# viiika/Diffusion-Conductor

Hardware: AMD Instinct MI355X
Metric: motion frames/sec (DDIM-50, 60s clip, bs=32 per GPU) (higher is better)
Workload: dtype f16; 1 GPU; configs[1]: DDIM-50 sampling loop, bs=32 clips/GPU x 1800 frames (60 s), linear attention, precision=fp16, conditioning + x_T resident in HBM (loop-only); clips_per_gpu=32, frames_per_clip=1800, ddim_steps=50, parallelism=clip-dp1, precise_tail_steps=1

## Files before the change

### diffusion-conductor_amd/csrc/dc_api.hip

```cpp
#include <hip/hip_runtime.h>

#include <algorithm>
#include <cmath>
#include <cstdarg>
#include <cstdio>
#include <cstdlib>
#include <cstring>
#include <map>
#include <string>
#include <tuple>
#include <vector>

#include "../../include/dc_ddim.h"
#include "dc_common.h"
#include "dc_form.h"
#include "dc_launch.h"
#include "dc_music.h"
#include "dc_pack.h"

namespace {

thread_local std::string g_err;

int fail(int code, const char* fmt, ...) {
// ... 639 lines not shown
int enqueue_step(dc_sampler* s, hipStream_t st, const Step& c, const Switches& w, StepDone* done = nullptr) {
    static const bool want_stamps = getenv("DC_STAMPS") != nullptr;
    const int B = s->B, T = s->T, M = s->M, G = s->G, Tx = s->Tx;
    const StepForm f = step_form(Geometry{B, T, Tx, G, s->num_cu, s->cap_rec_floats}, settings_of(s), w, c, want_stamps);
    const bool folded = f.folded;
    const int fs = f.fs, ff = f.ff, graph_step = c.graph_step;
    const bool ss = f.ss, sf = s->split_film;
    const unsigned l16_tag = folded ? 16u * (unsigned)graph_step : (0x40000000u | (16u * (s->l16_seq++ & 0x3ffffffu)));
    if (!f.error.empty()) return fail(DC_ERR_INVALID, "%s", f.error.c_str());
    if (done) done->embedded_next = f.embed_next, done->folded = folded;
    const DcModel* dmod = (c.split && !s->split_small) ? s->d_model_split : s->d_model;
    const int* iter_base = folded ? s->d_iter : nullptr;
    const int* t_src = folded ? s->d_t_of_iter + graph_step : s->d_t_clip;
    const float* coef_src = folded ? s->d_coef_of_iter + DC_COEF * (size_t)graph_step : s->d_coef_cur;
    const int* snap_src = folded ? s->d_snap_of_iter + graph_step : s->d_snap_cur;
    if (c.loop_mode && !folded)
        LAUNCH(K_BEGIN, dc_launch_begin_step(st, s->d_iter, s->d_t_of_iter, s->d_coef_of_t, s->d_snap_of_iter,
                                             s->d_t_clip, s->d_coef_cur, s->d_snap_cur, B));
    if (c.loop_mode && (s->upd_flags & DC_UPD_ZSTEP))
        LAUNCH(K_NOISE, dc_launch_step_noise(st, s->d_zstep, (size_t)B * Tx * s->cfg.input_feats, 0, reinterpret_cast<const unsigned long long*>(s->d_zslot) + 1,
                                             iter_base, folded ? graph_step : 0,
                                             folded ? nullptr : s->d_snap_cur, 0));
    if (!f.fuse_silu)
        LAUNCH(K_SILU, dc_launch_silu_emb(st, ff, sf, s->d_pp, s->h_model.temb, s->d_t_clip, s->d_s_hi, s->d_s_lo, G, T, B));
    DcEmbedArgs ea{};
    if (f.fuse_embed) ea = DcEmbedArgs{dmod, c.x_src, s->d_h, s->d_recs, s->d_length, M, Tx, f.nwg, f.upc, ss ? 1 : 0, 0};
    if (f.fuse_extra) ea = DcEmbedArgs{s->d_model, c.x_src, s->d_h, s->d_recs, s->d_length, M, Tx, f.nwg, f.upc, 0, 1};
    DcFilmArgs fa = film_args(s, f.fuse_silu ? s->d_pp : nullptr, t_src);
    if (f.g1_tiles) fa.bias_ft = s->h_model.film_b_g1, fa.bias16 = s->h_model.film_b16_g1;
    if (f.film_tail) fa.W16 = s->h_model.film_w16_tail;
    fa.clk = want_stamps ? s->d_stamps + 252 : nullptr;
    if (f.adapt) fa.rate_in = s->d_film_rate + 1024 * s->film_rate_parity, fa.rate_out = s->d_film_rate + 1024 * (s->film_rate_parity ^ 1);
    fa.iter_base = iter_base;
    fa.embed = (f.fuse_embed || f.fuse_extra) ? &ea : nullptr;
    const bool diag_skip_film = getenv("DC_DIAG_SKIP_FILM") && !f.fuse_embed && !f.fuse_extra && s->diag_film_done;
    s->diag_film_done = true;
    if (!diag_skip_film) LAUNCH(K_FILM, dc_launch_film_gemm(st, ff, sf, fa));
    s->film_rate_parity ^= 1;
    const int nl_run = f.nl_run;
    DcLayerArgs la{};
    la.dm = dmod, la.hbuf = s->d_h, la.E = s->d_E, la.NT = s->NT, la.recs = s->d_recs, la.length = s->d_length, la.xin = c.x_src, la.xout = c.x_dst;
    la.out_mode = c.loop_mode ? 1 : 0, la.coef_cur = coef_src, la.snap_cur = snap_src, la.snaps = s->d_snaps, la.iter_base = iter_base;
    la.M = M, la.T = T, la.G = G, la.B = B, la.Tx = Tx;
    la.upd = DcUpdate{s->d_zslot, s->d_status, (c.loop_mode ? s->upd_flags : 0) | f.upd_flags, folded ? graph_step : -1, nullptr};
    DcLayerArgs la_stamps = la;
    la_stamps.upd.stamps = s->d_stamps;
    if (s->cfg.no_eff) {
        LAUNCH(K_EMBED, dc_launch_embed_front_full(st, fs, ss, dmod, c.x_src, s->d_h, s->d_kv_sa[0], M, T, B, s->KT));
        for (int l = 0; l < nl_run; ++l)
            LAUNCH(K_LAYER, dc_launch_layer_full(st, fs, ss, (want_stamps && l == 3) ? la_stamps : la, l, s->d_kv_sa[l & 1], s->d_kv_sa[(l + 1) & 1],
                                                 s->d_kv_ca, s->KT, (l == nl_run - 1) ? f.stop_stage : 0));
        return DC_OK;
    }
    const DcLayerForm lf{fs, ss, f.wgr, f.narrow, f.g1_tiles, f.upc, f.rec_stride};
    if (f.fuse_embed || f.fuse_extra || c.embedded) {
    } else if (c.dbg.first >= 0)
        LAUNCH(K_EMBED, dc_launch_front_from_h(st, fs, ss, dmod, s->d_h, s->d_recs, s->d_length, M, T, G, B, c.dbg.first));
    else
        LAUNCH(K_EMBED, dc_launch_embed_front(st, lf, dmod, c.x_src, s->d_h, s->d_recs, s->d_length, M, T, G, B,
                                              want_stamps ? s->d_stamps + 256 : nullptr, Tx));
    for (int l = c.dbg.first >= 0 ? c.dbg.first : 0; l < nl_run; ++l) {
        if (f.layer16) {
            static const bool stamps16 = getenv("DC_L16_STAMPS") != nullptr;
            LAUNCH(K_LAYER, dc_launch_layer16(st, fs, (stamps16 && l == 3) ? la_stamps : la, l, s->d_a_ca16, f.upc16, f.rec_stride,
                                              l == 0 ? f.upc_narrow : f.upc16, l == 0 ? (size_t)2 * DC_REC_FLOATS : (size_t)DC_REC_FLOATS,
                                              f.l16_shared ? s->d_gran : nullptr, l16_tag, f.g1_tiles));
// ... 758 lines not shown
```

### diffusion-conductor_amd/csrc/dc_form.h

```cpp
#pragma once
#include <algorithm>
#include <cstdio>
#include <cstdlib>
#include <optional>
#include <string>

#include "dc_common.h"

constexpr int DCF_BF16 = 0, DCF_MIXED = 1, DCF_BF16X3 = 2, DCF_FP16 = 3;

struct Formats {
    int small_fmt = 0, film_fmt = 0;
    bool split_small = false, split_film = false;
    void set_precision(int precision) {
        split_small = precision == DCF_MIXED || precision == DCF_BF16X3;
        split_film = precision == DCF_BF16X3;
        small_fmt = precision == DCF_FP16 ? 1 : 0;
        film_fmt = (precision == DCF_FP16 || precision == DCF_MIXED) ? 1 : 0;
    }
};

#define DC_FORM_SWITCHES(X)                                                                                                            \
    X(no_wgrec, "DC_NO_WGREC") X(no_narrow, "DC_NO_NARROW") X(no_align, "DC_NO_ALIGN") X(align, "DC_ALIGN")                          \
    X(no_fuse_embed, "DC_NO_FUSE_EMBED") X(film_static, "DC_FILM_STATIC") X(begin_step, "DC_BEGIN_STEP") X(no_pad, "DC_NO_PAD")      \
    X(no_layer16, "DC_NO_LAYER16") X(l16_own_combine, "DC_L16_OWN_COMBINE") X(l16_test_drop_slice, "DC_L16_TEST_DROP_SLICE")         \
    X(tail_film_bf16, "DC_TAIL_FILM_BF16") X(flat_units, "DC_FLAT_UNITS") X(no_embed_next, "DC_NO_EMBED_NEXT")
struct Switches {
#define X(field, name) bool field = false;
    DC_FORM_SWITCHES(X)
#undef X
    static Switches read() {
        Switches w;
#define X(field, name) w.field = getenv(name) != nullptr;
        DC_FORM_SWITCHES(X)
#undef X
        return w;
    }
    unsigned long long bits() const {
        unsigned long long k = 0;
        int i = 0;
#define X(field, name) k |= (field ? 1ull : 0ull) << i++;
        DC_FORM_SWITCHES(X)
#undef X
        return k;
    }
};

inline size_t rec_capacity(size_t g) { return std::max(g * 2, 4 * ((g + 3) / 4) + 8) * DC_REC_FLOATS; }

struct Geometry {
    int B = 0, T = 0, Tx = 0, G = 0;
    int num_cu = 0;
    size_t cap_rec_floats = 0;
};

struct Settings {
    int precision = DCF_FP16;
    Formats fmt;
    bool no_eff = false;
    int clip_aligned = -1;
    bool l16_own = false;
    int num_layers = 0;
    bool split_model = false;
    bool film_w16 = false, film_w16_tail = false;
    int l16_max_units = 0;
};

struct Hooks {
    int layers = -1, stage = 0;
    int first = -1;
    bool production() const { return layers < 0 && stage == 0 && first < 0; }
};

struct StepOpts {
    bool loop_mode = false;
    int graph_step = -1;
    bool split = false;
    bool g1_loop = false;
    bool next_plain = false;
    bool embedded = false;
    bool profile = false;
    Hooks dbg;
};

struct StepForm {
    std::string error;
    bool ss = false;
    bool film_tail = false;
    int fs = 0, ff = 0;
    bool fuse_silu = false;
    bool folded = false;
    bool adapt = false;
    bool wgr = false, narrow = false, aligned = false, layer16 = false, l16_shared = false;
    int upc = 0, upc16 = 0, upc_narrow = 0, nwg = 0;
    size_t rec_stride = 0;
    bool mixed_form = false, embed_next = false, fuse_embed = false, fuse_extra = false, g1_tiles = false;
    int upd_flags = 0;
    int nl_run = 0, stop_stage = 0;
};

inline bool can_split_steps(const Settings& s, const Hooks& dbg) {
    return (s.precision == DCF_FP16 || s.precision == DCF_BF16) && dbg.production() && s.split_model;
}

inline StepForm step_form(const Geometry& g, const Settings& s, const Switches& w, const StepOpts& o, bool stamps) {
    StepForm f;
    const int B = g.B, T = g.T, G = g.G;
    const Hooks& dbg = o.dbg;
    const bool quiet = dbg.production() && !stamps;
    const bool ss = f.ss = s.fmt.split_small || o.split, sf = s.fmt.split_film;
    f.film_tail = o.split && !s.fmt.split_small && s.film_w16_tail && !w.tail_film_bf16;
    const int fs = f.fs = s.fmt.small_fmt, ff = f.ff = f.film_tail ? 1 : s.fmt.film_fmt;
    const bool fuse_silu = f.fuse_silu = !sf && dbg.layers < 0;
    f.folded = o.loop_mode && o.graph_step >= 0 && fuse_silu && !s.no_eff && !w.begin_step && dbg.stage == 0;
    f.adapt = !w.film_static && g.num_cu <= 1024;
    f.nl_run = (dbg.layers >= 0 && dbg.layers < s.num_layers) ? dbg.layers : s.num_layers;
    f.stop_stage = s.no_eff ? (dbg.stage ? dbg.stage : (f.nl_run < s.num_layers ? 3 : 0)) : dbg.stage;
    const bool wgr = f.wgr = T >= 256 && !w.no_wgrec && dbg.first < 0 && !s.no_eff && (!ss || (T % 32 == 0 && dbg.production() && !w.no_align));
    const bool can_align = wgr && T % 32 == 0 && !w.no_align;
    const int upc_wide = (T + 255) / 256, upc_narrow = f.upc_narrow = (T + 127) / 128;
    const bool aligned_env = can_align && w.align;
    const int nwg_narrow = can_align ? B * upc_narrow : (G + 3) / 4;
    const bool narrow = f.narrow = wgr && !ss && nwg_narrow <= g.num_cu && T <= 3840 && quiet && !w.no_narrow;
    const int nwg_flat = (G + 7) / 8, ncu = g.num_cu > 0 ? g.num_cu : 256;
    const bool same_rounds = ((long long)B * upc_wide + ncu - 1) / ncu == ((long long)nwg_flat + ncu - 1) / ncu;
    const bool aligned_wide = s.clip_aligned > 0 || aligned_env || (s.clip_aligned < 0 && same_rounds && !w.flat_units);
    const bool aligned = f.aligned = can_align && (narrow || ss || aligned_wide);
    const int upc16 = f.upc16 = (T + 63) / 64;
    const bool layer16 = f.layer16 = narrow && aligned && (long long)B * upc16 <= g.num_cu && upc16 <= s.l16_max_units && dbg.first < 0 && !w.no_layer16;
    const int upc = f.upc = aligned ? (narrow ? upc_narrow : upc_wide) : 0;
    const int nwg = f.nwg = aligned ? B * upc : (narrow ? (G + 3) / 4 : (G + 7) / 8);
    f.l16_shared = layer16 && !s.l16_own && !w.l16_own_combine;
    f.rec_stride = wgr ? (size_t)nwg * 2 * DC_REC_FLOATS : 0;
    const size_t rec_floats = wgr ? 2 * f.rec_stride : (size_t)G * 2 * DC_REC_FLOATS;
    if (rec_floats > g.cap_rec_floats) {
        char buf[160];
        snprintf(buf, sizeof buf, "unit records of this launch form (%zu floats) exceed the workspace (%zu)", rec_floats, g.cap_rec_floats);
        f.error = buf;
        return f;
    }
    const bool mixed_form = f.mixed_form = ss && !sf && ff == 1 && fs == 0;
    const bool wide_plain = wgr && !narrow && !ss && fuse_silu && ff == fs && quiet && !s.no_eff;
    f.embed_next = !w.no_embed_next && o.loop_mode && o.next_plain && wide_plain;
    if (o.embedded && !(o.loop_mode && wide_plain)) {
        f.error = "internal: a step whose front work was done by its predecessor changed its launch form";
        return f;
    }
    f.fuse_embed = !o.embedded && wgr && !narrow && (ss ? (aligned && mixed_form) : ff == fs) && fuse_silu && quiet && nwg <= g.num_cu &&
// ... 50 lines not shown
```

### diffusion-conductor_amd/csrc/dc_kernels.hip

```cpp
#include "dc_dev.h"


__global__ void k_begin_step(int* __restrict__ iter, const int* __restrict__ t_of_iter,
                             const float* __restrict__ coef_of_t, const int* __restrict__ snap_of_iter,
                             int* __restrict__ t_clip, float* __restrict__ coef_cur, int* __restrict__ snap_cur, int B) {
    const int it = *iter;
    const int t = t_of_iter[it];
    for (int b = threadIdx.x; b < B; b += blockDim.x) t_clip[b] = t;
    if (threadIdx.x < DC_COEF) coef_cur[threadIdx.x] = coef_of_t[t * DC_COEF + threadIdx.x];
    __syncthreads();
    if (threadIdx.x == 0) {
        snap_cur[0] = snap_of_iter ? snap_of_iter[it] : -1;
        snap_cur[1] = it;
        *iter = it + 1;
    }
}

__global__ void k_advance_iter(int* __restrict__ iter, int k) { *iter += k; }
__global__ void k_set_ptr(const float** slot, const float* p, unsigned long long seed, unsigned long long first) {
    slot[0] = p;
    reinterpret_cast<unsigned long long*>(slot)[1] = seed;
    reinterpret_cast<unsigned long long*>(slot)[2] = first;
}

// ... 612 lines not shown
#pragma unroll
    for (int m = 32; m >= 8; m >>= 1) cnt += __shfl_xor(cnt, m);
#pragma unroll
    for (int m = 32; m >= 1; m >>= 1) nzero += __shfl_xor(nzero, m);
    float tot = xsum;
#pragma unroll
    for (int m = 4; m >= 1; m >>= 1) tot += __shfl_xor(tot, m);
    const bool adaptive = rate_in && nzero == 0 && nw >= 64 && nunit >= 8ll * nw;
    int wx = 4096;
    if (adaptive) wx = (int)(fminf(fmaxf((xsum / (float)cnt) * ((float)nw / tot), 0.8f), 1.2f) * 4096.f + 0.5f);
    int before = 0, mine = 0, total = 0;
    for (int i = lane; i < nw; i += 64) {
        total += wx;
        before += i < b ? wx : 0;
        mine += i == b ? wx : 0;
    }
#pragma unroll
    for (int m = 32; m >= 1; m >>= 1) {
        total += __shfl_xor(total, m);
        before += __shfl_xor(before, m);
        mine += __shfl_xor(mine, m);
    }
    u0 = __builtin_amdgcn_readfirstlane((int)(nunit * before / total));
    u1 = __builtin_amdgcn_readfirstlane((int)(nunit * (before + mine) / total));
}

template <class T16>
DEV void film_gemm3_body(const v8<T16>* __restrict__ W, const float* __restrict__ bias16,
                         f16x16* __restrict__ E, int G, int NT, int round0, int nround,
                         const float* __restrict__ pp, const float* __restrict__ temb,
                         const int* __restrict__ t_clip, int T, int B,
                         unsigned long long* __restrict__ clk, const float* __restrict__ rate_in,
                         float* __restrict__ rate_out, const int* __restrict__ iter_base, unsigned long long t_begin,
                         int* __restrict__ status, int nw_film) {
    extern __shared__ __attribute__((aligned(16))) char lds[];
    using OP = v8<T16>;
#ifndef DC_FILM3_PF
#define DC_FILM3_PF 2
#endif
    constexpr int PF = DC_FILM3_PF;
    constexpr int KS = DC_E / 32;
    if (clk && blockIdx.x == 5 && threadIdx.x == 0) {
        clk[0] = __builtin_amdgcn_s_memtime();
        clk[1] = __builtin_amdgcn_s_memrealtime();
    }
    if (clk && threadIdx.x == 0 && blockIdx.x < 256) {
        clk[1036 + blockIdx.x * 4 + 0] = __builtin_amdgcn_s_memtime();
        clk[1036 + blockIdx.x * 4 + 1] = __builtin_amdgcn_s_memrealtime();
    }
    const int wave = threadIdx.x >> 6, lane = threadIdx.x & 63;
    const OP* slab = reinterpret_cast<const OP*>(lds);
    const int nblk = (G + 3) / 4;
    const long long nunit = (long long)nblk * nround;
    int u0, u1;
    film_shares(u0, u1, nunit, rate_in, lane, nw_film);
    OP a[PF][4];
    auto wpair = [&](int p) { return W + (size_t)(2 * p) * 2 * KS * 64 + lane; };
    auto wfrag = [&](const OP* w, int ks, int i) { return w[((size_t)(i >> 1) * 2 * KS + ks * 2 + (i & 1)) * 64]; };
    if (u0 < u1) {
        const OP* w0 = wpair((round0 + u0 % nround) * 8 + wave);
#pragma unroll
        for (int q = 0; q < PF; ++q)
#pragma unroll
            for (int i = 0; i < 4; ++i) a[q][i] = wfrag(w0, q, i);
    }
    int* pair_cnt = reinterpret_cast<int*>(lds + 4 * DC_KS_E * 1024);
    for (int useg = u0; useg < u1;) {
        const int tb = useg / nround, ra = useg % nround;
        const int nr = min(nround - ra, u1 - useg);
        const int npairs = nr * 8;
        const bool next_seg = useg + nr < u1;
        const int g0 = tb * 4;
        {
            v8<T16>* slab_w = reinterpret_cast<v8<T16>*>(lds);
            const float* trow[8];
#pragma unroll
            for (int i = 0; i < 8; ++i) {
                const int gg = min(g0 + (i >> 1), G - 1);
                const int b = min((gg * 32 + 16 * (i & 1) + (lane & 15)) / T, B - 1);
                trow[i] = temb + (size_t)t_clip[iter_base ? *iter_base : b] * 512 + 8 * (lane >> 4);
            }
#pragma unroll
            for (int half = 0; half < 2; ++half) {
                f32x8 pv[8], tv[8];
#pragma unroll
                for (int i = 0; i < 8; ++i) {
                    const int f = wave + 8 * (8 * half + i);
                    const int gi = 2 * half + (i >> 2), t16 = (f >> 4) & 1, ks = f & 15;
                    const int gg = min(g0 + gi, G - 1);
                    pv[i] = ld_pp(pp, (size_t)gg * DC_KS_E + 2 * ks + (lane >> 5), 32 * ((lane >> 4) & 1) + 16 * t16 + (lane & 15));
                    tv[i] = *reinterpret_cast<const f32x8*>(trow[2 * gi + t16] + 32 * ks);
                }
                __builtin_amdgcn_sched_barrier(0);
                if (half == 0) __syncthreads();
#pragma unroll
                for (int i = 0; i < 8; ++i) {
                    const int f = wave + 8 * (8 * half + i);
                    v8<T16> hi;
#pragma unroll
                    for (int j = 0; j < 4; ++j) {
                        const f32x2 z = silu_pair(pv[i][2 * j] + tv[i][2 * j], pv[i][2 * j + 1] + tv[i][2 * j + 1]);
                        hi[2 * j] = (T16)z.x;
                        hi[2 * j + 1] = (T16)z.y;
                    }
                    slab_w[f * 64 + lane] = hi;
                }
                __builtin_amdgcn_sched_barrier(0);
            }
            if (threadIdx.x == 0) *pair_cnt = 8;
            asm volatile("s_waitcnt vmcnt(0)" ::: "memory");
            __syncthreads();
        }
      for (int my = wave; my < npairs;) {
        int nxt = 0;
        if (lane == 0) nxt = __hip_atomic_fetch_add(pair_cnt, 1, __ATOMIC_RELAXED, __HIP_MEMORY_SCOPE_WORKGROUP);
        nxt = __builtin_amdgcn_readfirstlane(nxt);
        const int p = (round0 + ra + (my >> 3)) * 8 + (my & 7);
        const int ps = nxt < npairs ? (round0 + ra + (nxt >> 3)) * 8 + (nxt & 7) : (next_seg ? round0 * 8 + wave : p);
        const OP* w0 = wpair(p);
        const OP* wn = wpair(ps);
        f32x4 acc[2][2][4][2];
#pragma unroll
        for (int ti = 0; ti < 2; ++ti)
#pragma unroll
            for (int fb = 0; fb < 2; ++fb) {
                const f32x4 c = *reinterpret_cast<const f32x4*>(bias16 + (((size_t)(2 * p + ti) * 2 + fb) * 4 + (lane >> 4)) * 4);
#pragma unroll
                for (int g = 0; g < 4; ++g) acc[ti][fb][g][0] = acc[ti][fb][g][1] = c;
            }
        auto sfrag = [&](int gp, int i, int ks) { return slab[((size_t)((2 * gp + (i >> 1)) * 2 + (i & 1)) * KS + ks) * 64 + lane]; };
        OP bb[2][8];
#pragma unroll
        for (int i = 0; i < 8; ++i) bb[0][i] = sfrag(i >> 2, i & 3, 0);
#pragma unroll 1
        for (int ks0 = 0; ks0 < KS; ks0 += PF) {
            const bool tail = ks0 + PF >= KS;
#pragma unroll
            for (int q = 0; q < PF; ++q) {
                const int ks = ks0 + q, ksn = (ks + 1) & (KS - 1);
#pragma unroll
                for (int i = 0; i < 8; ++i) bb[(q + 1) & 1][i] = sfrag(i >> 2, i & 3, ksn);
#pragma unroll
                for (int k = 0; k < 4; ++k)
#pragma unroll
                    for (int i = 0; i < 8; ++i)
                        acc[k >> 1][k & 1][i >> 1][i & 1] = mfma16(a[q][k], bb[q & 1][i], acc[k >> 1][k & 1][i >> 1][i & 1]);
                __builtin_amdgcn_sched_barrier(0);
                {
                    const OP* src = tail ? wn : w0;
                    const int ksl = tail ? ks + PF - KS : ks + PF;
#pragma unroll
                    for (int i = 0; i < 4; ++i) a[q][i] = wfrag(src, ksl, i);
                }
                __builtin_amdgcn_sched_barrier(0);
            }
        }
        const int blk = p >> 2, t = p & 3;
#ifdef DC_FILM_SAT_CHECK
        {
            float am = 0.f;
#pragma unroll
            for (int ti = 0; ti < 2; ++ti)
#pragma unroll
                for (int fb = 0; fb < 2; ++fb)
#pragma unroll
                    for (int g = 0; g < 4; ++g) {
                        const f32x4 x = acc[ti][fb][g][0], y = acc[ti][fb][g][1];
                        am = absmax3(absmax3(absmax3(am, x[0], x[1]), x[2], x[3]), y[0], y[1]);
                        am = absmax3(am, y[2], y[3]);
                    }
            if (status && am > 65504.f) atomicOr(status, DC_STATUS_F16_SAT);
        }
#endif
#pragma unroll
        for (int g = 0; g < 4; ++g) {
            if (g0 + g >= G) continue;
#pragma unroll
            for (int ti = 0; ti < 2; ++ti) {
                u32x8 o;
#pragma unroll
                for (int fb = 0; fb < 2; ++fb)
#pragma unroll
                    for (int h2 = 0; h2 < 2; ++h2) {
                        const f32x4 x = acc[ti][fb][g][0], y = acc[ti][fb][g][1];
                        typedef _Float16 h2v __attribute__((ext_vector_type(2)));
                        const h2v xp = {(_Float16)x[2 * h2], (_Float16)x[2 * h2 + 1]}, yp = {(_Float16)y[2 * h2], (_Float16)y[2 * h2 + 1]};
                        const auto r = __builtin_amdgcn_permlane16_swap(__builtin_bit_cast(uint32_t, xp), __builtin_bit_cast(uint32_t, yp), false, false);
                        o[4 * fb + h2] = r[0];
                        o[4 * fb + 2 + h2] = r[1];
                    }
                store_etile(E, (size_t)(g0 + g) * NT + blk * 8 + 4 * ti + t, lane, __builtin_bit_cast(f16x16, o));
            }
        }
        my = nxt;
      }
        useg += nr;
    }
    if (clk && blockIdx.x == 5 && threadIdx.x == 0) {
        clk[2] = __builtin_amdgcn_s_memtime();
        clk[3] = __builtin_amdgcn_s_memrealtime();
    }
    if (clk && threadIdx.x == 0 && blockIdx.x < 256) {
        clk[1036 + blockIdx.x * 4 + 2] = __builtin_amdgcn_s_memtime();
        clk[1036 + blockIdx.x * 4 + 3] = __builtin_amdgcn_s_memrealtime();
        clk[1036 + 1024 + blockIdx.x] = (unsigned long long)(u1 - u0);
    }
    if (rate_out && threadIdx.x == 0) {
        const float ticks = (float)(long long)(__builtin_amdgcn_s_memrealtime() - t_begin);
        const float old = rate_in ? rate_in[blockIdx.x] : 0.f;
        const float now = (u1 > u0 && ticks > 0.f) ? (float)(u1 - u0) / ticks : 0.f;
        rate_out[blockIdx.x] = now > 0.f ? (old > 0.f ? 0.5f * old + 0.5f * now : now) : old;
    }
}
template <class T16>
__global__ __launch_bounds__(512, 2) void k_film_gemm3(const v8<T16>* __restrict__ W, const float* __restrict__ bias16,
                                                       f16x16* __restrict__ E, int G, int NT, int round0, int nround,
                                                       const float* __restrict__ pp, const float* __restrict__ temb,
                                                       const int* __restrict__ t_clip, int T, int B,
                                                       unsigned long long* __restrict__ clk, const float* __restrict__ rate_in,
                                                       float* __restrict__ rate_out, const int* __restrict__ iter_base,
                                                       int* __restrict__ status) {
    film_gemm3_body<T16>(W, bias16, E, G, NT, round0, nround, pp, temb, t_clip, T, B, clk, rate_in, rate_out, iter_base,
                         __builtin_amdgcn_s_memrealtime(), status, (int)gridDim.x);
}

template <class T16, bool SPLIT, bool WGR, bool FROMH = false, bool NARROW = false>
DEV void embed_front_body(const DcModel* __restrict__ dm, const float* __restrict__ x , float* __restrict__ hbuf,
                          float* __restrict__ recs, const int* __restrict__ length, int M, int T, int G, int B,
                          unsigned long long* __restrict__ clk , int l0,
                          int Tx ,
                          int upc ,
                          int wg_fixed ) {
    static_assert(!(FROMH && WGR), "the h-injection hook exists for the per-group-record form only");
    static_assert(!NARROW || (WGR && !SPLIT), "narrow workgroups exist for the workgroup-record form of the non-split formats");
    constexpr int NW = (NARROW || (SPLIT && !WGR)) ? 4 : 8;
    constexpr int WM = SPLIT ? 2 : 1;
    const bool stamping = clk && blockIdx.x == 100 && threadIdx.x == 0;
    auto stamp = [&](int i) {
        if (stamping) clk[i] = __builtin_amdgcn_s_memrealtime();
    };
    stamp(0);
    using W = v8<T16>;
    const int wave = threadIdx.x >> 6, lane = threadIdx.x & 63;
    const int wg = wg_fixed >= 0 ? wg_fixed : (WGR ? wg_index() : (int)blockIdx.x);
    const WgMap wm = wg_map(wg, wave, NW, G, M, T, B, WGR ? upc : 0);
    const int g = wm.g;
    const bool active = wm.active;
    const GroupCtx cx = make_ctx(g, lane, M, T);
    const int P = dm->input_feats;
    const int xb = min(cx.tok, M - 1) / T, xn = cx.tok - xb * T;
    const bool live = cx.tok < M && xn < Tx;
    const int n = live ? xn : 0;
    const size_t xrow = (size_t)xb * Tx + n;
    extern __shared__ __attribute__((aligned(16))) char lds[];
    constexpr int NIMG = 32 * WM + 1;
    constexpr int PST_SZ = SPLIT ? NIMG * 1024 : 65536, XP_SZ = SPLIT ? 0 : 8192;
// ... 109 lines not shown
            mmb_oc<4, 4, T16, SPLIT>(V, lv, oc, nf, lane);
            float ssum;
            f32x8 keep;
            partial_tile<T16, SPLIT>(K[oc], V, vr_own, wg_colmax<NW>(mx, oc, s0, cx.c), cx, ssum, keep);
            pst[(wave * 4 + oc) * 64 + lane] = keep;
            if (cx.hh == 0) ss[(wave * 4 + oc) * 32 + cx.c] = ssum;
            if (!SPLIT && active && cx.straddle) {
                partial_tile<T16, SPLIT>(K[oc], V, vr[1], wg_colmax<NW>(mx, oc, 1, cx.c), cx, ssum, keep);
                xp[oc * 64 + lane] = keep;
                if (cx.hh == 0) ss[(NW * 4 + oc) * 32 + cx.c] = ssum;
            }
            __builtin_amdgcn_sched_barrier(0);
        }
        stamp(5);
        __syncthreads();
        stamp(6);
        wg_write_record<NW>(recs, mx, pst, xp, ss, wave, lane, ub0, wm.nact, wm.Mu, wm.Tu, wg);
        stamp(7);
    }
}
template <class T16, bool SPLIT, bool WGR, bool FROMH = false, bool NARROW = false>
__global__ __launch_bounds__((NARROW || (SPLIT && !WGR)) ? 256 : 512, (SPLIT && !WGR) ? 1 : 2)
void k_embed_front(const DcModel* __restrict__ dm, const float* __restrict__ x, float* __restrict__ hbuf, float* __restrict__ recs,
                   const int* __restrict__ length, int M, int T, int G, int B, unsigned long long* __restrict__ clk, int l0, int Tx, int upc) {
    embed_front_body<T16, SPLIT, WGR, FROMH, NARROW>(dm, x, hbuf, recs, length, M, T, G, B, clk, l0, Tx, upc, -1);
}
template <class T16, class TS = T16, bool SP = false>
__global__ __launch_bounds__(512, 2) void k_film_embed(const v8<T16>* __restrict__ W, const float* __restrict__ bias16,
                                                       f16x16* __restrict__ E, int G, int NT, int round0, int nround,
                                                       const float* __restrict__ pp, const float* __restrict__ temb,
                                                       const int* __restrict__ t_clip, int T, int B,
                                                       unsigned long long* __restrict__ clk, const float* __restrict__ rate_in,
                                                       float* __restrict__ rate_out, const int* __restrict__ iter_base, const DcEmbedArgs ea,
                                                       int* __restrict__ status) {
    const unsigned long long t_begin = __builtin_amdgcn_s_memrealtime();
    if constexpr (!SP) {
        if (ea.extra) {
            const int nf = (int)gridDim.x - ea.ne;
            if ((int)blockIdx.x >= nf) {
                if (threadIdx.x >= 256) return;
                embed_front_body<TS, false, true, false, true>(ea.dm, ea.x, ea.hbuf, ea.recs, ea.length, ea.M, T, G, B, nullptr, 0, ea.Tx, ea.upc,
                                                               (int)blockIdx.x - nf);
                return;
            }
            film_gemm3_body<T16>(W, bias16, E, G, NT, round0, nround, pp, temb, t_clip, T, B, clk, rate_in, rate_out, iter_base, t_begin, status, nf);
            return;
        }
    }
    if ((int)blockIdx.x < ea.ne) {
        embed_front_body<TS, SP, true, false, false>(ea.dm, ea.x, ea.hbuf, ea.recs, ea.length, ea.M, T, G, B, nullptr, 0, ea.Tx, ea.upc,
                                                     (int)blockIdx.x);
        asm volatile("s_waitcnt vmcnt(0) lgkmcnt(0)" ::: "memory");
        __syncthreads();
    }
    film_gemm3_body<T16>(W, bias16, E, G, NT, round0, nround, pp, temb, t_clip, T, B, clk, rate_in, rate_out, iter_base, t_begin, status,
                         (int)gridDim.x);
}

#ifndef DC_SPLIT_STYL_PF
#define DC_SPLIT_STYL_PF 2
#endif
#ifndef DC_SPLIT_NW
#define DC_SPLIT_NW 8
#endif
template <class T16, bool SPLIT, bool DBG, bool STAMP, bool WGR, bool NARROW = false, bool G1 = false >
__global__ __launch_bounds__((NARROW || (SPLIT && DC_SPLIT_NW == 4)) ? 256 : 512, (SPLIT && DC_SPLIT_NW == 4) ? 1 : 2)
void k_layer(const DcModel* __restrict__ dm, int l, float* __restrict__ hbuf, const f16x16* __restrict__ E, int NT,
             const v8<T16>* __restrict__ a_sa , const v8<T16>* __restrict__ a_ca ,
             float* __restrict__ recs, const int* __restrict__ length, const float* __restrict__ xin,
             float* __restrict__ xout, int out_mode, const float* __restrict__ coef_cur, const int* __restrict__ snap_cur,
             float* __restrict__ snaps, int M, int T, int G, int B, int dbg,
             unsigned long long* __restrict__ stamps, size_t rec_stride, const int* __restrict__ iter_base,
             int Tx , int upc ,
             const DcUpdate upd) {
    extern __shared__ __attribute__((aligned(16))) char lds[];
    static_assert(!NARROW || (WGR && !SPLIT && !DBG), "narrow workgroups: workgroup-record form, non-split formats, no test hooks");
    constexpr int NW = NARROW ? 4 : (SPLIT ? DC_SPLIT_NW : 8);
    constexpr int WM = SPLIT ? 2 : 1;
    constexpr int NFW = 32 * WM;
#define DC_STAMP(k)                                                                                        \
    do {                                                                                                   \
        if (STAMP && stamps && blockIdx.x == 3 && (threadIdx.x & 63) == 0 && l == 3)                       \
            stamps[(threadIdx.x >> 6) * 32 + (k)] = __builtin_amdgcn_s_memrealtime();                      \
    } while (0)
#define DC_WGSTAMP(e)                                                                                      \
    do {                                                                                                   \
        if (STAMP && stamps && threadIdx.x == 0 && (l == 3 || l == 4) && blockIdx.x < 256)                 \
            stamps[264 + ((l - 3) * 256 + blockIdx.x) * 2 + (e)] = __builtin_amdgcn_s_memrealtime();       \
    } while (0)
// ... 1356 lines not shown
    k_film_gemm<T16, SP><<<dim3(a.NT / 8, (a.G + 3) / 4), dim3(256), 0, st>>>((const v8<T16>*)a.W, a.bias_ft, (const v8<T16>*)a.s_hi,
                                                                             (const v8<T16>*)a.s_lo, (f16x16*)a.E, a.G, a.NT, a.status);
}
static int film_extra_workgroups(long long nunit, int nblk, int ne, int ncu) {
    const int room = ncu - ne;
    const long long alone = nunit < ncu ? nunit : ncu;
    if (room >= nblk && room >= 1) {
        const int nf = (int)(nunit < room ? nunit : room);
        if ((nunit + nf - 1) / nf == (nunit + alone - 1) / alone) return nf;
    }
    return (int)alone;
}
template <class T16>
static hipError_t launch_film3_t(hipStream_t st, const DcFilmArgs& a) {
    const size_t shm = 4 * DC_KS_E * 1024 + 64;
    static unsigned long long optin_done = 0;
    if (hipError_t e = lds_optin((const void*)k_film_gemm3<T16>, (int)shm, optin_done)) return e;
    const int ncu = cu_count();
    const int nblk = (a.G + 3) / 4;
    const long long nunit = (long long)nblk * a.nround;
    int nwg = (int)(nunit < ncu ? nunit : ncu);
    if (nwg < nblk) nwg = nblk < ncu ? nblk : ncu;
    if (nwg < 1) nwg = 1;
    const v8<T16>* W16 = (const v8<T16>*)a.W16;
    f16x16* E = (f16x16*)a.E;
    const DcEmbedArgs* ea = a.embed;
    if (ea && ea->x && ea->extra) {
        if (ea->split_bf16 || ea->upc <= 0) return hipErrorInvalidValue;
        const int nf = film_extra_workgroups(nunit, nblk, ea->ne, ncu);
        if (nf <= 0) return hipErrorInvalidValue;
        static unsigned long long optin4 = 0;
        if (hipError_t e = lds_optin((const void*)k_film_embed<T16>, (int)shm, optin4)) return e;
        k_film_embed<T16><<<dim3(nf + ea->ne), dim3(512), shm, st>>>(W16, a.bias16, E, a.G, a.NT, a.round0, a.nround, a.pp, a.temb, a.t_clip, a.T,
                                                                     a.B, a.clk, a.rate_in, a.rate_out, a.iter_base, *ea, a.status);
        return hipGetLastError();
    }
    if (ea && ea->x && nwg >= ea->ne) {
        if (ea->split_bf16) {
            if (!std::is_same<T16, _Float16>::value || ea->upc <= 0) return hipErrorInvalidValue;
            const size_t shm2 = 8192 + 65 * 1024 + 9 * 4 * 32 * 4 + 65 * 1024;
            static unsigned long long optin3 = 0;
            if (hipError_t e = lds_optin((const void*)k_film_embed<T16, __bf16, true>, (int)shm2, optin3)) return e;
            k_film_embed<T16, __bf16, true><<<dim3(nwg), dim3(512), shm2, st>>>(W16, a.bias16, E, a.G, a.NT, a.round0, a.nround, a.pp, a.temb,
                                                                                a.t_clip, a.T, a.B, a.clk, a.rate_in, a.rate_out, a.iter_base, *ea,
                                                                                a.status);
            return hipGetLastError();
        }
        static unsigned long long optin2 = 0;
        if (hipError_t e = lds_optin((const void*)k_film_embed<T16>, (int)shm, optin2)) return e;
        k_film_embed<T16><<<dim3(nwg), dim3(512), shm, st>>>(W16, a.bias16, E, a.G, a.NT, a.round0, a.nround, a.pp, a.temb, a.t_clip, a.T, a.B,
                                                             a.clk, a.rate_in, a.rate_out, a.iter_base, *ea, a.status);
        return hipGetLastError();
    }
    if (ea && ea->x) return hipErrorInvalidValue;
    k_film_gemm3<T16><<<dim3(nwg), dim3(512), shm, st>>>(W16, a.bias16, E, a.G, a.NT, a.round0, a.nround, a.pp, a.temb, a.t_clip, a.T, a.B,
                                                         a.clk, a.rate_in, a.rate_out, a.iter_base, a.status);
    return hipGetLastError();
}
hipError_t dc_launch_film_gemm(hipStream_t st, int fmt, bool split, const DcFilmArgs& a) {
    if (!split && a.pp && a.W16) return fmt == 1 ? launch_film3_t<_Float16>(st, a) : launch_film3_t<__bf16>(st, a);
    if (a.embed && a.embed->x) return hipErrorInvalidValue;
    if (a.round0 != 0) return hipSuccess;
    DISPATCH(fmt, split, (launch_film_t<T16, SP>(st, a)));
    return LAUNCH_CHECK();
}

template <class T16, bool SP>
static hipError_t launch_front_from_h_t(hipStream_t st, const DcModel* dm, float* hbuf, float* recs, const int* length,
                                        int M, int T, int G, int B, int l0) {
    constexpr int NW = SP ? 4 : 8;
    k_embed_front<T16, SP, false, true><<<dim3((G + NW - 1) / NW), dim3(NW * 64), 0, st>>>(dm, nullptr, hbuf, recs, length, M, T, G, B, nullptr, l0, T, 0);
    return hipGetLastError();
}
hipError_t dc_launch_front_from_h(hipStream_t st, int fmt, bool split, const DcModel* dm, float* hbuf, float* recs, const int* length,
                                  int M, int T, int G, int B, int l0) {
    hipError_t e = hipSuccess;
    DISPATCH(fmt, split, (e = launch_front_from_h_t<T16, SP>(st, dm, hbuf, recs, length, M, T, G, B, l0)));
    return e;
}

template <class T16, bool SP, bool WGR, bool NARROW = false>
static hipError_t launch_embed_t(hipStream_t st, const DcModel* dm, const float* x, float* hbuf, float* recs, const int* length,
                                 int M, int T, int G, int B, unsigned long long* clk, int Tx, int upc) {
    constexpr int NW = (NARROW || (SP && !WGR)) ? 4 : 8;
    const size_t shm = !WGR ? 0 : SP ? 8192 + 65 * 1024 + 9 * 4 * 32 * 4 + 65 * 1024 : 8192 + 65536 + 8192 + 9 * 4 * 32 * 4 + 33 * 1024;
    if (WGR) {
        static unsigned long long optin_done = 0;
        if (hipError_t e = lds_optin((const void*)k_embed_front<T16, SP, WGR, false, NARROW>, (int)shm, optin_done)) return e;
    }
// ... 114 lines not shown
```

### diffusion-conductor_amd/csrc/dc_launch.h

```cpp
#pragma once
#include <hip/hip_runtime.h>
#include "dc_common.h"

hipError_t dc_launch_begin_step(hipStream_t st, int* iter, const int* t_of_iter, const float* coef_of_t,
                                const int* snap_of_iter, int* t_clip, float* coef_cur, int* snap_cur, int B);
hipError_t dc_launch_temb_table(hipStream_t st, const float* freqs, const float* w0t, const float* b0,
                                const float* w2t, const float* b2, float* temb, int nt);
hipError_t dc_launch_cond_embed(hipStream_t st, int mode, const float* xf, const float* wt, const float* b, float* out_f32,
                                void* out_hi, void* out_lo, int M, int G, int T ,
                                int Tx );
hipError_t dc_launch_ca_partials(hipStream_t st, const DcModel* dm, const void* nh_hi, const void* nh_lo,
                                 float* recs, int M, int T, int G, int L, int Tx );
hipError_t dc_launch_cond_pp64(hipStream_t st, const float* xf , const void* wpack, const float* b, float* out_f32, int M, int G, int T, int Tx);
hipError_t dc_launch_ca_partials64(hipStream_t st, const DcModel* dm, const float* xf , const float* gram, float* rstd, float* recs,
                                   int M, int T, int G, int L, int Tx);
hipError_t dc_launch_attn_combine(hipStream_t st, int fmt, const float* recs, void* afrag, int T, int NU, int B, int nset,
                                  int gran);
hipError_t dc_launch_silu_emb(hipStream_t st, int fmt, bool split, const float* pp, const float* temb, const int* t_clip,
                              void* s_hi, void* s_lo, int G, int T, int B,
                              const int* iter_base = nullptr );
struct DcFilmArgs {
    const void* W;
    const float* bias_ft;
    const void *s_hi, *s_lo;
    void* E;
    int G, NT, round0, nround;
    const float *pp, *temb;
    const int* t_clip;
    int T, B;
    unsigned long long* clk;
    const float* rate_in;
    float* rate_out;
    const int* iter_base;
    const void* W16;
    const float* bias16;
    const DcEmbedArgs* embed;
    int* status;
};
hipError_t dc_launch_film_gemm(hipStream_t st, int fmt, bool split, const DcFilmArgs& a);
struct DcLayerForm {
    int fmt;
    bool split;
    bool wgr;
    bool narrow;
    bool g1;
    int upc;
    size_t rec_stride;
};
hipError_t dc_launch_embed_front(hipStream_t st, const DcLayerForm& f, const DcModel* dm, const float* x, float* hbuf, float* recs,
                                 const int* length, int M, int T, int G, int B,
                                 unsigned long long* clk ,
                                 int Tx );
hipError_t dc_launch_front_from_h(hipStream_t st, int fmt, bool split, const DcModel* dm, float* hbuf, float* recs, const int* length,
                                  int M, int T, int G, int B, int l0);
struct DcLayerArgs {
    const DcModel* dm;
    float* hbuf;
    const void* E;
    int NT;
    float* recs;
    const int* length;
    const float* xin;
    float* xout;
    int out_mode;
    const float* coef_cur;
    const int* snap_cur;
    float* snaps;
    const int* iter_base;
    int M, T, G, B;
    int Tx;
// ... 30 lines not shown
```

Baseline: 1.625 million frames/s.

## Prefetch next FiLM slab fill during tail of current segment and interleave fill loads

Restructures the FiLM GEMM slab fill (SiLU of pp+temb into LDS) into helper lambdas that interleave loads and writes in a software-pipelined order. When a wave draws the last pair of a segment and another segment follows, it starts loading the next segment's pp values before its epilogue stores and then performs the fill, so the next fill overlaps the current work. An env switch restores the serial fill ordering. This adds register pressure and more complex barrier logic inside the pair loop, which could hurt occupancy.

```diff
diff --git a/diffusion-conductor_amd/csrc/dc_api.hip b/diffusion-conductor_amd/csrc/dc_api.hip
--- a/diffusion-conductor_amd/csrc/dc_api.hip
+++ b/diffusion-conductor_amd/csrc/dc_api.hip
@@ -695,6 +695,7 @@
     fa.clk = want_stamps ? s->d_stamps + 252 : nullptr;
     if (f.adapt) fa.rate_in = s->d_film_rate + 1024 * s->film_rate_parity, fa.rate_out = s->d_film_rate + 1024 * (s->film_rate_parity ^ 1);
     fa.iter_base = iter_base;
+    fa.fill_serial = f.fill_serial;
     fa.embed = (f.fuse_embed || f.fuse_extra) ? &ea : nullptr;
     const bool diag_skip_film = getenv("DC_DIAG_SKIP_FILM") && !f.fuse_embed && !f.fuse_extra && s->diag_film_done;
     s->diag_film_done = true;
diff --git a/diffusion-conductor_amd/csrc/dc_form.h b/diffusion-conductor_amd/csrc/dc_form.h
--- a/diffusion-conductor_amd/csrc/dc_form.h
+++ b/diffusion-conductor_amd/csrc/dc_form.h
@@ -24,7 +24,8 @@
     X(no_wgrec, "DC_NO_WGREC") X(no_narrow, "DC_NO_NARROW") X(no_align, "DC_NO_ALIGN") X(align, "DC_ALIGN")                          \
     X(no_fuse_embed, "DC_NO_FUSE_EMBED") X(film_static, "DC_FILM_STATIC") X(begin_step, "DC_BEGIN_STEP") X(no_pad, "DC_NO_PAD")      \
     X(no_layer16, "DC_NO_LAYER16") X(l16_own_combine, "DC_L16_OWN_COMBINE") X(l16_test_drop_slice, "DC_L16_TEST_DROP_SLICE")         \
-    X(tail_film_bf16, "DC_TAIL_FILM_BF16") X(flat_units, "DC_FLAT_UNITS") X(no_embed_next, "DC_NO_EMBED_NEXT")
+    X(tail_film_bf16, "DC_TAIL_FILM_BF16") X(flat_units, "DC_FLAT_UNITS") X(no_embed_next, "DC_NO_EMBED_NEXT")       \
+    X(film_fill_serial, "DC_FILM_FILL_SERIAL")
 struct Switches {
 #define X(field, name) bool field = false;
     DC_FORM_SWITCHES(X)
@@ -91,6 +92,7 @@
     bool fuse_silu = false;
     bool folded = false;
     bool adapt = false;
+    bool fill_serial = false;
     bool wgr = false, narrow = false, aligned = false, layer16 = false, l16_shared = false;
     int upc = 0, upc16 = 0, upc_narrow = 0, nwg = 0;
     size_t rec_stride = 0;
@@ -114,6 +116,7 @@
     const bool fuse_silu = f.fuse_silu = !sf && dbg.layers < 0;
     f.folded = o.loop_mode && o.graph_step >= 0 && fuse_silu && !s.no_eff && !w.begin_step && dbg.stage == 0;
     f.adapt = !w.film_static && g.num_cu <= 1024;
+    f.fill_serial = w.film_fill_serial;
     f.nl_run = (dbg.layers >= 0 && dbg.layers < s.num_layers) ? dbg.layers : s.num_layers;
     f.stop_stage = s.no_eff ? (dbg.stage ? dbg.stage : (f.nl_run < s.num_layers ? 3 : 0)) : dbg.stage;
     const bool wgr = f.wgr = T >= 256 && !w.no_wgrec && dbg.first < 0 && !s.no_eff && (!ss || (T % 32 == 0 && dbg.production() && !w.no_align));
diff --git a/diffusion-conductor_amd/csrc/dc_kernels.hip b/diffusion-conductor_amd/csrc/dc_kernels.hip
--- a/diffusion-conductor_amd/csrc/dc_kernels.hip
+++ b/diffusion-conductor_amd/csrc/dc_kernels.hip
@@ -668,7 +668,7 @@
                          const int* __restrict__ t_clip, int T, int B,
                          unsigned long long* __restrict__ clk, const float* __restrict__ rate_in,
                          float* __restrict__ rate_out, const int* __restrict__ iter_base, unsigned long long t_begin,
-                         int* __restrict__ status, int nw_film) {
+                         int* __restrict__ status, int nw_film, int fill_serial ) {
     extern __shared__ __attribute__((aligned(16))) char lds[];
     using OP = v8<T16>;
 #ifndef DC_FILM3_PF
@@ -701,52 +701,102 @@
             for (int i = 0; i < 4; ++i) a[q][i] = wfrag(w0, q, i);
     }
     int* pair_cnt = reinterpret_cast<int*>(lds + 4 * DC_KS_E * 1024);
+    v8<T16>* const slab_w = reinterpret_cast<v8<T16>*>(lds);
+    const int ws = __builtin_amdgcn_readfirstlane(wave);
+    const int ib = iter_base ? *iter_base : -1;
+    auto fill_lane = [&]() {
+        int ln = lane;
+        asm volatile("" : "+v"(ln));
+        return ln;
+    };
+    auto fill_row = [&](int g0, int i, int ln) {
+        int idx = ib;
+        if (ib < 0) idx = min((min(g0 + (i >> 1), G - 1) * 32 + 16 * (i & 1) + (ln & 15)) / T, B - 1);
+        return (uint32_t)((t_clip[idx] * 512 + 8 * (ln >> 4) + 32 * ws) * 4);
+    };
+    auto fill_load_pv = [&](f32x8 (&pv)[4], int g0, int q, int ln) {
+        const int gg = __builtin_amdgcn_readfirstlane(min(g0 + q, G - 1));
+        const char* const pq = reinterpret_cast<const char*>(pp) + (size_t)gg * (DC_KS_E * 128 * 16) + (size_t)ws * (2 * 128 * 16);
+        const uint32_t pp_lane = (uint32_t)(((ln >> 5) * 128 + 32 * ((ln >> 4) & 1) + (ln & 15)) * 16);
+#pragma unroll
+        for (int i = 0; i < 4; ++i) {
+            const char* const p = pq + (i & 1) * (16 * 128 * 16) + (i >> 1) * 256 + pp_lane;
+            const f32x4 lo = *reinterpret_cast<const f32x4*>(p), hi = *reinterpret_cast<const f32x4*>(p + 1024);
+#pragma unroll
+            for (int j = 0; j < 4; ++j) pv[i][j] = lo[j], pv[i][4 + j] = hi[j];
+        }
+    };
+    auto fill_load_tv = [&](f32x8 (&tv)[4], uint32_t row0, uint32_t row1) {
+#pragma unroll
+        for (int i = 0; i < 4; ++i)
+            tv[i] = *reinterpret_cast<const f32x8*>(reinterpret_cast<const char*>(temb) + (i & 1) * (8 * 32 * 4) + ((i >> 1) ? row1 : row0));
+    };
+    auto fill_write = [&](const f32x8 (&pv)[4], const f32x8 (&tv)[4], int q, int ln) {
+#pragma unroll
+        for (int i = 0; i < 4; ++i) {
+            const int f = ws + 8 * (4 * q + i);
+            v8<T16> hi;
+#pragma unroll
+            for (int j = 0; j < 4; ++j) {
+                const f32x2 z = silu_pair(pv[i][2 * j] + tv[i][2 * j], pv[i][2 * j + 1] + tv[i][2 * j + 1]);
+                hi[2 * j] = (T16)z.x;
+                hi[2 * j + 1] = (T16)z.y;
+            }
+            slab_w[f * 64 + ln] = hi;
+        }
+    };
+    auto fill_rest = [&](f32x8 (&pvA)[4], int g0, bool serial) {
+        const int ln = fill_lane();
+        uint32_t row[8];
+#pragma unroll
+        for (int i = 0; i < 8; ++i) row[i] = fill_row(g0, i, ln);
+        f32x8 tvA[4], pvB[4], tvB[4];
+        fill_load_pv(pvB, g0, 1, ln);
+        fill_load_tv(tvA, row[0], row[1]);
+        fill_load_tv(tvB, row[2], row[3]);
+        __builtin_amdgcn_sched_barrier(0);
+        __syncthreads();
+        fill_write(pvA, tvA, 0, ln);
+        __builtin_amdgcn_sched_barrier(0);
+        if (serial) {
+            fill_write(pvB, tvB, 1, ln);
+            __builtin_amdgcn_sched_barrier(0);
+            fill_load_pv(pvA, g0, 2, ln);
+            fill_load_tv(tvA, row[4], row[5]);
+            fill_load_pv(pvB, g0, 3, ln);
+            fill_load_tv(tvB, row[6], row[7]);
+        } else {
+            fill_load_pv(pvA, g0, 2, ln);
+            fill_load_tv(tvA, row[4], row[5]);
+            __builtin_amdgcn_sched_barrier(0);
+            fill_write(pvB, tvB, 1, ln);
+            __builtin_amdgcn_sched_barrier(0);
+            fill_load_pv(pvB, g0, 3, ln);
+            fill_load_tv(tvB, row[6], row[7]);
+        }
+        __builtin_amdgcn_sched_barrier(0);
+        fill_write(pvA, tvA, 2, ln);
+        __builtin_amdgcn_sched_barrier(0);
+        fill_write(pvB, tvB, 3, ln);
+        __builtin_amdgcn_sched_barrier(0);
+        if (threadIdx.x == 0) *pair_cnt = 8;
+        asm volatile("s_waitcnt vmcnt(0)" ::: "memory");
+        __syncthreads();
+    };
+    bool filled = false;
     for (int useg = u0; useg < u1;) {
         const int tb = useg / nround, ra = useg % nround;
         const int nr = min(nround - ra, u1 - useg);
         const int npairs = nr * 8;
         const bool next_seg = useg + nr < u1;
         const int g0 = tb * 4;
-        {
-            v8<T16>* slab_w = reinterpret_cast<v8<T16>*>(lds);
-            const float* trow[8];
-#pragma unroll
-            for (int i = 0; i < 8; ++i) {
-                const int gg = min(g0 + (i >> 1), G - 1);
-                const int b = min((gg * 32 + 16 * (i & 1) + (lane & 15)) / T, B - 1);
-                trow[i] = temb + (size_t)t_clip[iter_base ? *iter_base : b] * 512 + 8 * (lane >> 4);
-            }
-#pragma unroll
-            for (int half = 0; half < 2; ++half) {
-                f32x8 pv[8], tv[8];
-#pragma unroll
-                for (int i = 0; i < 8; ++i) {
-                    const int f = wave + 8 * (8 * half + i);
-                    const int gi = 2 * half + (i >> 2), t16 = (f >> 4) & 1, ks = f & 15;
-                    const int gg = min(g0 + gi, G - 1);
-                    pv[i] = ld_pp(pp, (size_t)gg * DC_KS_E + 2 * ks + (lane >> 5), 32 * ((lane >> 4) & 1) + 16 * t16 + (lane & 15));
-                    tv[i] = *reinterpret_cast<const f32x8*>(trow[2 * gi + t16] + 32 * ks);
-                }
-                __builtin_amdgcn_sched_barrier(0);
-                if (half == 0) __syncthreads();
-#pragma unroll
-                for (int i = 0; i < 8; ++i) {
-                    const int f = wave + 8 * (8 * half + i);
-                    v8<T16> hi;
-#pragma unroll
-                    for (int j = 0; j < 4; ++j) {
-                        const f32x2 z = silu_pair(pv[i][2 * j] + tv[i][2 * j], pv[i][2 * j + 1] + tv[i][2 * j + 1]);
-                        hi[2 * j] = (T16)z.x;
-                        hi[2 * j + 1] = (T16)z.y;
-                    }
-                    slab_w[f * 64 + lane] = hi;
-                }
-                __builtin_amdgcn_sched_barrier(0);
-            }
-            if (threadIdx.x == 0) *pair_cnt = 8;
-            asm volatile("s_waitcnt vmcnt(0)" ::: "memory");
-            __syncthreads();
-        }
+        if (!filled) {
+            f32x8 pvA[4];
+            fill_load_pv(pvA, g0, 0, fill_lane());
+            __builtin_amdgcn_sched_barrier(0);
+            fill_rest(pvA, g0, fill_serial != 0);
+        }
+        filled = false;
       for (int my = wave; my < npairs;) {
         int nxt = 0;
         if (lane == 0) nxt = __hip_atomic_fetch_add(pair_cnt, 1, __ATOMIC_RELAXED, __HIP_MEMORY_SCOPE_WORKGROUP);
@@ -791,6 +841,10 @@
                 __builtin_amdgcn_sched_barrier(0);
             }
         }
+        const bool pre = !fill_serial && next_seg && nxt >= npairs;
+        f32x8 pvA[4];
+        if (pre) fill_load_pv(pvA, g0 + 4, 0, fill_lane());
+        __builtin_amdgcn_sched_barrier(0);
         const int blk = p >> 2, t = p & 3;
 #ifdef DC_FILM_SAT_CHECK
         {
@@ -828,6 +882,11 @@
                 store_etile(E, (size_t)(g0 + g) * NT + blk * 8 + 4 * ti + t, lane, __builtin_bit_cast(f16x16, o));
             }
         }
+        if (pre) {
+            __builtin_amdgcn_sched_barrier(0);
+            fill_rest(pvA, g0 + 4, false);
+            filled = true;
+        }
         my = nxt;
       }
         useg += nr;
@@ -855,9 +914,9 @@
                                                        const int* __restrict__ t_clip, int T, int B,
                                                        unsigned long long* __restrict__ clk, const float* __restrict__ rate_in,
                                                        float* __restrict__ rate_out, const int* __restrict__ iter_base,
-                                                       int* __restrict__ status) {
+                                                       int* __restrict__ status, int fill_serial) {
     film_gemm3_body<T16>(W, bias16, E, G, NT, round0, nround, pp, temb, t_clip, T, B, clk, rate_in, rate_out, iter_base,
-                         __builtin_amdgcn_s_memrealtime(), status, (int)gridDim.x);
+                         __builtin_amdgcn_s_memrealtime(), status, (int)gridDim.x, fill_serial);
 }
 
 template <class T16, bool SPLIT, bool WGR, bool FROMH = false, bool NARROW = false>
@@ -1033,7 +1092,7 @@
                                                        const int* __restrict__ t_clip, int T, int B,
                                                        unsigned long long* __restrict__ clk, const float* __restrict__ rate_in,
                                                        float* __restrict__ rate_out, const int* __restrict__ iter_base, const DcEmbedArgs ea,
-                                                       int* __restrict__ status) {
+                                                       int* __restrict__ status, int fill_serial) {
     const unsigned long long t_begin = __builtin_amdgcn_s_memrealtime();
     if constexpr (!SP) {
         if (ea.extra) {
@@ -1044,7 +1103,7 @@
                                                                (int)blockIdx.x - nf);
                 return;
             }
-            film_gemm3_body<T16>(W, bias16, E, G, NT, round0, nround, pp, temb, t_clip, T, B, clk, rate_in, rate_out, iter_base, t_begin, status, nf);
+            film_gemm3_body<T16>(W, bias16, E, G, NT, round0, nround, pp, temb, t_clip, T, B, clk, rate_in, rate_out, iter_base, t_begin, status, nf, fill_serial);
             return;
         }
     }
@@ -1055,7 +1114,7 @@
         __syncthreads();
     }
     film_gemm3_body<T16>(W, bias16, E, G, NT, round0, nround, pp, temb, t_clip, T, B, clk, rate_in, rate_out, iter_base, t_begin, status,
-                         (int)gridDim.x);
+                         (int)gridDim.x, fill_serial);
 }
 
 #ifndef DC_SPLIT_STYL_PF
@@ -2478,7 +2537,7 @@
         static unsigned long long optin4 = 0;
         if (hipError_t e = lds_optin((const void*)k_film_embed<T16>, (int)shm, optin4)) return e;
         k_film_embed<T16><<<dim3(nf + ea->ne), dim3(512), shm, st>>>(W16, a.bias16, E, a.G, a.NT, a.round0, a.nround, a.pp, a.temb, a.t_clip, a.T,
-                                                                     a.B, a.clk, a.rate_in, a.rate_out, a.iter_base, *ea, a.status);
+                                                                     a.B, a.clk, a.rate_in, a.rate_out, a.iter_base, *ea, a.status, a.fill_serial ? 1 : 0);
         return hipGetLastError();
     }
     if (ea && ea->x && nwg >= ea->ne) {
@@ -2489,18 +2548,18 @@
             if (hipError_t e = lds_optin((const void*)k_film_embed<T16, __bf16, true>, (int)shm2, optin3)) return e;
             k_film_embed<T16, __bf16, true><<<dim3(nwg), dim3(512), shm2, st>>>(W16, a.bias16, E, a.G, a.NT, a.round0, a.nround, a.pp, a.temb,
                                                                                 a.t_clip, a.T, a.B, a.clk, a.rate_in, a.rate_out, a.iter_base, *ea,
-                                                                                a.status);
+                                                                                a.status, a.fill_serial ? 1 : 0);
             return hipGetLastError();
         }
         static unsigned long long optin2 = 0;
         if (hipError_t e = lds_optin((const void*)k_film_embed<T16>, (int)shm, optin2)) return e;
         k_film_embed<T16><<<dim3(nwg), dim3(512), shm, st>>>(W16, a.bias16, E, a.G, a.NT, a.round0, a.nround, a.pp, a.temb, a.t_clip, a.T, a.B,
-                                                             a.clk, a.rate_in, a.rate_out, a.iter_base, *ea, a.status);
+                                                             a.clk, a.rate_in, a.rate_out, a.iter_base, *ea, a.status, a.fill_serial ? 1 : 0);
         return hipGetLastError();
     }
     if (ea && ea->x) return hipErrorInvalidValue;
     k_film_gemm3<T16><<<dim3(nwg), dim3(512), shm, st>>>(W16, a.bias16, E, a.G, a.NT, a.round0, a.nround, a.pp, a.temb, a.t_clip, a.T, a.B,
-                                                         a.clk, a.rate_in, a.rate_out, a.iter_base, a.status);
+                                                         a.clk, a.rate_in, a.rate_out, a.iter_base, a.status, a.fill_serial ? 1 : 0);
     return hipGetLastError();
 }
 hipError_t dc_launch_film_gemm(hipStream_t st, int fmt, bool split, const DcFilmArgs& a) {
diff --git a/diffusion-conductor_amd/csrc/dc_launch.h b/diffusion-conductor_amd/csrc/dc_launch.h
--- a/diffusion-conductor_amd/csrc/dc_launch.h
+++ b/diffusion-conductor_amd/csrc/dc_launch.h
@@ -36,6 +36,7 @@
     const float* bias16;
     const DcEmbedArgs* embed;
     int* status;
+    bool fill_serial;
 };
 hipError_t dc_launch_film_gemm(hipStream_t st, int fmt, bool split, const DcFilmArgs& a);
 struct DcLayerForm {
```

Result: no change. 1.627 million frames/s, median of 5 (+0.1%).
